# matwilso/generative_models

Measured on AMD Instinct MI355X. Metric: ddpm_train_images_per_sec, higher is better.
Workload: dtype fp16_fwd+bf16_bwd

## Files before the change

### generative_models_amd/csrc/conv_halo.hip

```cpp
#include "gmk_common.h"


namespace {

typedef __attribute__((ext_vector_type(4))) unsigned int u32x4;
typedef __attribute__((ext_vector_type(2))) unsigned int u32x2_t;

constexpr int kHaloSlots = 448;
constexpr int kHB = kHaloSlots * 128;
constexpr int kWOFF = 2 * kHB;
constexpr int kWST = 16384;

struct HaloParams {
    const void* src0; const void* src1;
    int c0, c1, ktot;
    int B, H, W, WE, R, TP, ntiles, rows_total;
    int nfull, nhalf;
    int shift;
    int pmask;
    const void* w; unsigned w_tap_stride_b; int n0;
    const float* bias; const float* emb; int emb_stride;
    const void* residual; void* out; int out_cstride; int M;
    unsigned nb0, nb1, nbw, nbo;
    const float* gn_scale; const float* gn_shift; int gn_stride;
// ... 1514 lines not shown
                if (tap < 8) pre(hbuf, tap + 1);
                if (tap == 8 && ph + 1 == nph) b_off = next_boff;
                if (kPrefetchW) load_wt(st, 0, 0);
                mfma_group(1, IntTag<0>{});
                if (tap < 8) interleave_pre();
                __builtin_amdgcn_sched_barrier(0);
            }
            hbuf ^= 1;
        };
        phase(IntTag<1>{}, 0);
        for (int ph = 1; ph < nph; ++ph) phase(IntTag<0>{}, ph);
        asm volatile("" ::: "memory");
        if (hand) {
            Rl = smem + (hbuf ^ 1) * HB;
            if (cwe == 1) {
#pragma unroll
                for (int i = 0; i < 4; ++i) {
                    const int ml = pxbase + i * 32 + r;
                    const int m = tile * p.TP + ml;
                    const unsigned off = (ml < p.TP && m < p.M) ? (unsigned)m * (unsigned)p.out_cstride * ES + (unsigned)(nblk + 112 + 8 * h) * ES : kBadOff;
                    r7[i] = __builtin_bit_cast(u32x4, __builtin_amdgcn_raw_buffer_load_b128(rsr, off, 0, 0));
                }
            }
            __builtin_amdgcn_s_barrier();
            __builtin_amdgcn_s_barrier();
        }
        epilogue();
    };

    set_geometry(job_half(0));
    b_off = WOFF + (cwe * 64 + r) * 128;
    resolve_centres(job_tile(0));
#pragma unroll
    for (int j = 0; j < 2; ++j)
#pragma unroll
        for (int i = 0; i < 4; ++i)
#pragma unroll
            for (int e = 0; e < 16; ++e) acc[j][i][e] = 0.f;
    __builtin_amdgcn_s_barrier();
    if (kPrefetchW) load_wt(0, 0, 0);
    for (int k = 0; k < njobs; ++k) {
        const int tile = job_tile(k), hc = job_half(k), ntile = job_tile(k + 1), nhc = job_half(k + 1);
        const int next_boff = WOFF + ((nhc >= 0 ? nhc : cw) * 64 + r) * 128;
        if (hc < 0) run_job(IntTag<4>{}, tile, next_boff);
        else run_job(IntTag<2>{}, tile, next_boff);
        if (nhc != hc) set_geometry(nhc);
        resolve_centres(ntile);
        asm volatile("" ::: "memory");
    }
}

}

static unsigned* g_stamps = nullptr;
static int64_t g_stamp_bytes = 0;
extern "C" int gmk_dev_set_stamp_buffer(void* buf, int64_t bytes) { g_stamps = (unsigned*)buf; g_stamp_bytes = bytes; return 0; }

int gmk_halo_geometry(int B, int H, int W, int c0, int c1, int w_rows, int cout, int out_cstride, int min_tiles, int upsample,
                      int fused_gn, HaloGeometry* g) {
    if (c0 % 64 || c1 % 64 || cout % 128) return 0;
    if (c1 != 0 && c1 != c0) return 0;
    if (W < 4 || W > 254 || H < 2) return 0;
    const int R = 256 / W;
    if (R < 1) return 0;
    const int crossings = H % R == 0 ? 0 : (R - 1 + H - 1) / H;
    const int ner = R + 2 + 2 * crossings;
    if (ner * (W + 2) > kHaloSlots) return 0;
    const int64_t rows_total = (int64_t)B * H;
    const int64_t M = rows_total * W;
    if (upsample && ((H | W) & 1)) return 0;
    const int64_t Msrc = upsample ? M / 4 : M;
    const int64_t nb0 = Msrc * c0 * 2, nb1 = Msrc * c1 * 2;
    const int64_t nbw = (int64_t)9 * w_rows * (c0 + c1) * 2, nbo = M * out_cstride * 2;
    const int64_t lim = 0xFFFF0000ll;
    if (nb0 >= lim || nb1 >= lim || nbw >= lim || nbo >= lim || M >= 0x00FFFFFF || c0 > 2048 || c1 > 2048) return 0;
    const int64_t ntiles = (rows_total + R - 1) / R;
    if (ntiles < min_tiles) return 0;
    if (fused_gn && (upsample || R > H)) return 0;
    if (g) {
        g->R = R; g->TP = R * W; g->slots = ner * (W + 1) + 1; g->rows_total = rows_total; g->M = M; g->ntiles = ntiles;
        g->nb0 = nb0; g->nb1 = nb1; g->nbw = nbw; g->nbo = nbo;
    }
    return 1;
}

int gmk_conv3x3_halo_try(const void* src0, const void* src1, int c0, int c1, int B, int H, int W, const void* w, int w_rows,
                         int n0, int cout, const float* bias, const float* emb, int emb_stride, const void* residual,
                         void* out, int out_cstride, int min_tiles, int upsample, float* stats, int64_t stats_bytes,
                         const float* gn_scale, const float* gn_shift, int gn_stride, int dtype, hipStream_t stream) {
    HaloGeometry g;
    if (!gmk_halo_geometry(B, H, W, c0, c1, w_rows, cout, out_cstride, min_tiles, upsample, gn_scale != nullptr, &g)) return 0;
    if (gn_scale && (!gn_shift || gn_stride < c0 + c1)) return 0;
    const int R = g.R, TP = g.TP;
    const int64_t rows_total = g.rows_total, M = g.M, ntiles = g.ntiles;
    const int64_t nb0 = g.nb0, nb1 = g.nb1, nbw = g.nbw, nbo = g.nbo;
    HaloParams p;
    p.src0 = src0; p.src1 = src1; p.c0 = c0; p.c1 = c1; p.ktot = c0 + c1;
    p.shift = upsample ? 1 : 0; p.pmask = upsample == 2 ? 1 : 0;
    p.B = B; p.H = H; p.W = W; p.WE = W + 1; p.R = R; p.TP = TP; p.ntiles = (int)ntiles; p.rows_total = (int)rows_total;
    p.w = w; p.w_tap_stride_b = (unsigned)w_rows * (unsigned)(c0 + c1) * 2u; p.n0 = n0;
    p.bias = bias; p.emb = emb; p.emb_stride = emb_stride; p.residual = residual; p.out = out; p.out_cstride = out_cstride;
    p.M = (int)M;
    p.nb0 = (unsigned)nb0; p.nb1 = (unsigned)nb1; p.nbw = (unsigned)nbw; p.nbo = (unsigned)nbo;
    p.gn_scale = gn_scale; p.gn_shift = gn_shift; p.gn_stride = gn_stride;
    p.stats = nullptr; p.stats_groups = out_cstride / 4; p.stamps = nullptr;
    p.variant = gmk_kernel_choice(3, "GMK_DEV_VARIANT") & 0xFF;
    if (stats && cout == out_cstride && stats_bytes >= ntiles * 8 * 2 * (int64_t)(out_cstride / 4) * 2 * 4 && H * W >= 32) p.stats = stats;
    p.inv_hp2 = 1.0f / (float)(H + 2); p.inv_h = 1.0f / (float)H; p.inv_we = 1.0f / (float)(W + 1); p.inv_w = 1.0f / (float)W;
    const int ncu = gmk_cu_limit();
// ... 93 lines not shown
```

### generative_models_amd/csrc/gmk_common.h

```cpp
#pragma once
#include <hip/hip_runtime.h>
#include <stdint.h>

#include "../../include/gmk.h"

typedef __bf16 bf16_t;
typedef __attribute__((ext_vector_type(8))) __bf16 bf16x8;
typedef __attribute__((ext_vector_type(4))) __bf16 bf16x4;
typedef _Float16 f16_t;
typedef __attribute__((ext_vector_type(8))) _Float16 f16x8;
typedef __attribute__((ext_vector_type(4))) _Float16 f16x4;
typedef __attribute__((ext_vector_type(2))) _Float16 f16x2;
typedef __attribute__((ext_vector_type(2))) __bf16 bf16x2;
typedef __attribute__((ext_vector_type(4))) short s16x4;
typedef __attribute__((ext_vector_type(4))) float f32x4;
typedef __attribute__((ext_vector_type(16))) float f32x16;

#define GMK_LDS __attribute__((address_space(3)))

void gmk_set_error(const char* fmt, ...);
int gmk_check_launch(const char* what);
int gmk_kernel_choice(int which, const char* env);
int gmk_conv1x1_pair_stream_try(const void* src, int64_t npix, const void* w_rows256, void* out_a, void* out_b, int dtype, hipStream_t stream);
int gmk_conv1x1_wgrad_stream_try(const void* dy, int dy_cstride, const void* src0, const void* src1, int64_t npix, float* slab, int64_t slab_bytes,
                                 bool x_f16, hipStream_t stream);
int gmk_conv_subpixel_takes(int B, int H, int W, int cin, int cout, int w_rows, int ntaps, int out_cstride, int dtype);
bool fp32_split(void);
int gmk_cu_limit(void);
void gmk_note_kernel(int id);

#define GMK_REQUIRE(cond, ...)                 \
    do {                                       \
        if (!(cond)) {                         \
            gmk_set_error(__VA_ARGS__);        \
            return GMK_ERR_ARG;                \
        }                                      \
    } while (0)

int gmk_conv3x3_halo_try(const void* src0, const void* src1, int c0, int c1, int B, int H, int W, const void* w, int w_rows,
                         int n0, int cout, const float* bias, const float* emb, int emb_stride, const void* residual,
                         void* out, int out_cstride, int min_tiles, int upsample, float* stats, int64_t stats_bytes,
                         const float* gn_scale, const float* gn_shift, int gn_stride, int dtype, hipStream_t stream);

struct HaloGeometry { int R, TP, slots; int64_t rows_total, M, ntiles, nb0, nb1, nbw, nbo; };
int gmk_halo_geometry(int B, int H, int W, int c0, int c1, int w_rows, int cout, int out_cstride, int min_tiles, int upsample,
                      int fused_gn, HaloGeometry* g);

int gmk_wgrad_slots_nsplit(int cout, int ktot);
int gmk_conv_wgrad_slots_try(const void* dy, int dy_cstride, const void* src0, const void* src1, int c0, int c1, int B, int H,
                             int W, int cout, float* slab, int64_t slab_bytes, int forced, int upsample, bool x_f16,
                             hipStream_t stream, int stride2 = 0);


static inline hipStream_t gmk_stream(void* s) { return reinterpret_cast<hipStream_t>(s); }
static inline int gmk_esize(int dtype) { return dtype == GMK_F32 ? 4 : 2; }
static inline bool gmk_is16(int dtype) { return dtype == GMK_BF16 || dtype == GMK_F16; }

template <typename T> struct Vec8;

__device__ __forceinline__ void load8(const float* p, float (&v)[8]) {
    const f32x4 a = *reinterpret_cast<const f32x4*>(p);
    const f32x4 b = *reinterpret_cast<const f32x4*>(p + 4);
    v[0] = a[0]; v[1] = a[1]; v[2] = a[2]; v[3] = a[3];
    v[4] = b[0]; v[5] = b[1]; v[6] = b[2]; v[7] = b[3];
}
__device__ __forceinline__ void load8(const bf16_t* p, float (&v)[8]) {
    const bf16x8 a = *reinterpret_cast<const bf16x8*>(p);
#pragma unroll
    for (int i = 0; i < 8; ++i) v[i] = (float)a[i];
}
__device__ __forceinline__ void load8(const f16_t* p, float (&v)[8]) {
    const f16x8 a = *reinterpret_cast<const f16x8*>(p);
#pragma unroll
    for (int i = 0; i < 8; ++i) v[i] = (float)a[i];
}
__device__ __forceinline__ void store8(float* p, const float (&v)[8]) {
    f32x4 a = {v[0], v[1], v[2], v[3]}, b = {v[4], v[5], v[6], v[7]};
    *reinterpret_cast<f32x4*>(p) = a;
    *reinterpret_cast<f32x4*>(p + 4) = b;
}
__device__ __forceinline__ void store8(bf16_t* p, const float (&v)[8]) {
    bf16x8 a;
// ... 121 lines not shown
```

### generative_models_amd/csrc/gmk_common.hip

```cpp
#include <stdarg.h>
#include <stdio.h>
#include <stdlib.h>

#include "gmk_common.h"

static thread_local char g_err[512] = "";

void gmk_set_error(const char* fmt, ...) {
    va_list ap;
    va_start(ap, fmt);
    vsnprintf(g_err, sizeof(g_err), fmt, ap);
    va_end(ap);
}

int gmk_check_launch(const char* what) {
    hipError_t e = hipGetLastError();
    if (e != hipSuccess) {
        gmk_set_error("%s: %s", what, hipGetErrorString(e));
        return (int)e;
    }
    return 0;
}

extern "C" int gmk_version(void) { return 1; }
extern "C" const char* gmk_last_error(void) { return g_err; }

static thread_local int g_last_kernel = 0;
void gmk_note_kernel(int id) { g_last_kernel = id; }
extern "C" int gmk_last_kernel(void) { return g_last_kernel; }

static int g_choice[4] = {-1, -1, -1, -1};
extern "C" int gmk_set_kernel_choice(int conv, int wgrad, int gn) {
    g_choice[0] = conv; g_choice[1] = wgrad; g_choice[2] = gn;
    return 0;
}
extern "C" int gmk_set_dev_variant(int v) { g_choice[3] = v; return 0; }
int gmk_kernel_choice(int which, const char* env) {
    if (g_choice[which] >= 0) return g_choice[which];
    const char* v = getenv(env);
    return v ? atoi(v) : 0;
}

static int g_cu_limit = -1;
extern "C" int gmk_set_cu_limit(int n) {
    if (n < 8 || n > 256) { gmk_set_error("gmk_set_cu_limit: %d not in [8, 256]", n); return GMK_ERR_ARG; }
    g_cu_limit = n;
    return 0;
}
int gmk_cu_limit(void) {
    if (g_cu_limit > 0) return g_cu_limit;
    const char* v = getenv("GMK_CU_LIMIT");
    const int n = v ? atoi(v) : 256;
    return n >= 8 && n <= 256 ? n : 256;
}
extern "C" int gmk_get_cu_limit(void) { return gmk_cu_limit(); }

static int g_fp32_exact = -1;
extern "C" int gmk_set_fp32_exact(int exact) { g_fp32_exact = exact ? 1 : 0; return 0; }
bool fp32_split(void) {
    if (g_fp32_exact < 0) {
        const char* v = getenv("GMK_FP32_SPLIT");
        g_fp32_exact = (v && atoi(v) != 0) ? 0 : 1;
    }
    return g_fp32_exact == 0;
}
extern "C" int gmk_fp32_split(void) { return fp32_split() ? 1 : 0; }
```

### generative_models_amd/csrc/gn_silu.hip

```cpp
#include <stdlib.h>

#include "gmk_common.h"

namespace {

constexpr int kThreads = 256;

__device__ __forceinline__ void drop8(float (&v)[8], size_t e0, float p, uint64_t seed, uint64_t off) {
    const float scale = 1.0f / (1.0f - p);
#pragma unroll
    for (int q = 0; q < 2; ++q) {
        uint32_t r[4];
        philox4x32(off + (uint64_t)(e0 >> 2) + q, seed, r);
#pragma unroll
        for (int k = 0; k < 4; ++k) v[4 * q + k] = u01(r[k]) >= p ? v[4 * q + k] * scale : 0.f;
    }
}

__device__ __forceinline__ void slab_of_block(int idx, int nslab, int B, int& b, int& slab) {
    if ((B & 7) == 0) {
        const int xcd = idx & 7, j = idx >> 3;
        slab = j % nslab;
        b = (j / nslab) * 8 + xcd;
    } else {
// ... 578 lines not shown
    } else
#pragma unroll
    for (int i = 0; i < ITER; ++i, eoff += estride, loff += PL * NVEC * 16) {
        if (ITER > 8) asm volatile("" : "+v"(eoff), "+v"(loff));
        const int p = pl + PL * i;
        if (!kExact && p >= HW) continue;
        const size_t off = eoff;
        const u32x4_t xr = i >= XLDS ? xk[i >= XLDS ? i - XLDS : 0] : *reinterpret_cast<const u32x4_t*>(xs_lds + loff);
        const u32x4_t dq2 = i < KEEP ? dr[i < KEEP ? i : 0] : *reinterpret_cast<const u32x4_t*>(dy + off);
        float o[8];
#pragma unroll
        for (int jj = 0; jj < 4; ++jj) {
            const f32x2_t xv = unpack2<TX>(xr[jj]), dv = unpack2<bf16_t>(dq2[jj]);
            const f32x2_t dg = silu_grad2(xv, dv, sv[jj], tv[jj], kNegLog2e);
            const f32x2_t ov = __builtin_elementwise_fma(dg, sv[jj], __builtin_elementwise_fma(xv, npv[jj], qv[jj]));
            o[2 * jj] = ov[0]; o[2 * jj + 1] = ov[1];
        }
        if (dadd1) {
            float t[8];
            load8(dadd1 + off, t);
#pragma unroll
            for (int k = 0; k < 8; ++k) o[k] += t[k];
        }
        if (dadd2) {
            float t[8];
            load8(dadd2 + off, t);
#pragma unroll
            for (int k = 0; k < 8; ++k) o[k] += t[k];
        }
#pragma unroll
        for (int k = 0; k < 8; ++k) xs[k] += o[k];
        store8(dx + off, o);
        if (i & 1) __builtin_amdgcn_sched_barrier(0);
    }
    if (dxsum) {
#pragma unroll
        for (int k = 0; k < 8; ++k) xs[k] = vec_lane_sum<NVEC>(xs[k]);
        __syncthreads();
        if (lane < NVEC) {
#pragma unroll
            for (int k = 0; k < 8; ++k) red[wave][lane][k] = xs[k];
        }
        __syncthreads();
        if (tid < CS) {
            const int vv = tid >> 3, k = tid & 7;
            float a = 0.f;
#pragma unroll
            for (int w = 0; w < NW; ++w) a += red[w][vv][k];
            dxsum[(size_t)b * dxsum_stride + c0 + tid] = a;
        }
    }
}

int gn_reg_iter(int HW, int nvec) {
    if (nvec == 8 && HW == 784 && gmk_kernel_choice(2, "GMK_GN_KERNEL") != 6) return 14;
    for (int it = 1; it <= 16; it <<= 1)
        if (((HW + it - 1) / it) * nvec <= 512) return it;
    return 0;
}


template <typename T>
__global__ __launch_bounds__(kThreads) void chansum_kernel(const T* __restrict__ x, float* __restrict__ out,
                                                          int out_stride, int HW, int C) {
    __shared__ float red[kThreads * 8];
    const int b = blockIdx.x, tid = threadIdx.x;
    const int nvec = C >> 3, planes = kThreads / nvec;
    const int vec = tid % nvec, pl = tid / nvec;
    const T* xb = x + (size_t)b * HW * C + vec * 8;
    float s[8];
#pragma unroll
    for (int i = 0; i < 8; ++i) s[i] = 0.f;
    for (int p = pl; p < HW; p += planes) {
        float v[8];
        load8(xb + (size_t)p * C, v);
#pragma unroll
        for (int i = 0; i < 8; ++i) s[i] += v[i];
    }
#pragma unroll
    for (int i = 0; i < 8; ++i) red[tid * 8 + i] = s[i];
    __syncthreads();
    if (tid < C) {
        const int vv = tid >> 3, i = tid & 7;
        float a = 0.f;
        for (int p = 0; p < planes; ++p) a += red[(p * nvec + vv) * 8 + i];
        out[(size_t)b * out_stride + tid] = a;
    }
}

__global__ __launch_bounds__(256) void colsum_kernel(const float* __restrict__ part, int64_t stride,
                                                    float* __restrict__ out, int R, int C, int accumulate) {
    __shared__ float red[8][33];
    const int cl = threadIdx.x & 31, rl = threadIdx.x >> 5;
    const int c = blockIdx.x * 32 + cl;
    float s = 0.f;
    if (c < C) {
        float s0 = 0.f, s1 = 0.f, s2 = 0.f, s3 = 0.f;
        int r = rl;
        for (; r + 24 < R; r += 32) {
            s0 += part[(int64_t)r * stride + c];
            s1 += part[(int64_t)(r + 8) * stride + c];
            s2 += part[(int64_t)(r + 16) * stride + c];
            s3 += part[(int64_t)(r + 24) * stride + c];
        }
        for (; r < R; r += 8) s0 += part[(int64_t)r * stride + c];
        s = (s0 + s1) + (s2 + s3);
// ... 32 lines not shown
        load8(p00 + (int64_t)2 * W * C + C, t);
#pragma unroll
        for (int i = 0; i < 8; ++i) a[i] += t[i];
        store8(y + ((b * H + oy) * W + ox) * (int64_t)C + vec * 8, a);
    }
}

template <typename TS, typename TD>
__global__ __launch_bounds__(256) void cast16_kernel(const TS* __restrict__ src, TD* __restrict__ dst, int64_t nvec) {
    fp16_saturating_stores<TD>();
    for (int64_t i = (int64_t)blockIdx.x * 256 + threadIdx.x; i < nvec; i += (int64_t)gridDim.x * 256) {
        float v[8];
        load8(src + i * 8, v);
#pragma unroll
        for (int k = 0; k < 8; ++k) v[k] = sat16<TD>(v[k]);
        store8(dst + i * 8, v);
    }
}

bool gn_shape_ok(int C, int G) {
    if (C <= 0 || C > 256 || (C & 7) || 256 % (C >> 3)) return false;
    if (G < 0) return -G >= 1 && -G <= 16;
    if (G <= 0 || G > 256 || C % G) return false;
    const int cpg = C / G;
    return cpg == 1 || cpg == 2 || cpg == 4 || cpg == 8 || cpg == 16;
}
static bool gn_narrow(int C, int G) { return G < 0 || C / G < 4; }

int gn_slab_channels(int mode, int C, int G, int HW, int elem_bytes, bool backward) {
    if (G < 0) return C;
    const int cpg = C / G;
    int CS = C;
    if (mode == 3) CS = 32;
    else if (mode == 4) CS = 64;
    else if (mode != 1) CS = backward && (int64_t)HW * C * elem_bytes > 65536 ? 32 : C;
    if (CS > C || C % CS || CS % cpg || (CS & 7) || kThreads % (CS >> 3)) CS = C;
    return CS;
}

}

extern "C" int gmk_gn_silu_fwd(const void* x, void* y, const float* gamma, const float* beta, float* mean, float* rstd,
                               int B, int HW, int C, int groups, float eps, const float* stats_part, int tile_pixels,
                               int ntiles, float drop_p, uint64_t drop_seed, uint64_t drop_offset, const float* xadd,
                               int xadd_stride, int dtype, void* stream) {
    GMK_REQUIRE(!xadd || xadd_stride >= C, "gmk_gn_silu_fwd: xadd_stride %d < C %d", xadd_stride, C);
    if (xadd) stats_part = nullptr;
    GMK_REQUIRE(drop_p >= 0.f && drop_p < 1.f, "gmk_gn_silu_fwd: dropout probability %g outside [0, 1)", (double)drop_p);
    GMK_REQUIRE(!stats_part || (tile_pixels >= 32 && ntiles > 0 && HW >= 32 && C % 4 == 0),
                "gmk_gn_silu_fwd: bad statistics geometry");
    GMK_REQUIRE(x && y && gamma && beta && mean && rstd, "gmk_gn_silu_fwd: null pointer");
    GMK_REQUIRE(B > 0 && HW > 0 && gn_shape_ok(C, groups), "gmk_gn_silu_fwd: unsupported shape B=%d HW=%d C=%d G=%d", B,
                HW, C, groups);
    const int gn_mode = gmk_kernel_choice(2, "GMK_GN_KERNEL");
    GMK_REQUIRE(dtype != GMK_F16 || !stats_part, "gmk_gn_silu_fwd: producer statistics go with bf16 tensors only");
    if (gn_narrow(C, groups)) {
        GMK_REQUIRE(!stats_part, "gmk_gn_silu_fwd: producer statistics come in 4-channel units; groups of %d channels", groups < 0 ? -groups : C / groups);
        gmk_note_kernel(22);
        if (dtype == GMK_BF16)
            gn_silu_fwd_kernel<bf16_t, true><<<B, kThreads, 0, gmk_stream(stream)>>>((const bf16_t*)x, (bf16_t*)y, gamma, beta, mean, rstd, HW, C, groups,
                                                                                   eps, nullptr, 0, 0, C, B, drop_p, drop_seed, drop_offset, xadd, xadd_stride);
        else if (dtype == GMK_F16)
            gn_silu_fwd_kernel<f16_t, true><<<B, kThreads, 0, gmk_stream(stream)>>>((const f16_t*)x, (f16_t*)y, gamma, beta, mean, rstd, HW, C, groups,
                                                                                  eps, nullptr, 0, 0, C, B, drop_p, drop_seed, drop_offset, xadd, xadd_stride);
        else if (dtype == GMK_F32)
            gn_silu_fwd_kernel<float, true><<<B, kThreads, 0, gmk_stream(stream)>>>((const float*)x, (float*)y, gamma, beta, mean, rstd, HW, C, groups,
                                                                                  eps, nullptr, 0, 0, C, B, drop_p, drop_seed, drop_offset, xadd, xadd_stride);
        else
            GMK_REQUIRE(false, "gmk_gn_silu_fwd: bad dtype %d", dtype);
        return gmk_check_launch("gmk_gn_silu_fwd");
    }
    const bool big = gmk_is16(dtype) && !stats_part && (gn_mode == 8 || gn_mode == 0) && HW > 1024 && HW <= 4096 && HW % 16 == 0 &&
                     C % 32 == 0 && 32 % (C / groups) == 0;
    if (big || (gmk_is16(dtype) && !stats_part && (gn_mode == 5 || gn_mode == 6 || (gn_mode == 0 && HW > 64)) && C % 64 == 0 &&
               32 % (C / groups) == 0 && gn_reg_iter(HW, 8) > 0)) {
        const int nvec = (big || gn_mode == 5) ? 4 : 8;
        const int it = big ? 16 : gn_reg_iter(HW, nvec), planes = (HW + it - 1) / it, threads = (planes * nvec + 63) / 64 * 64;
        const int nblk = B * (C / (nvec * 8));
        gmk_note_kernel(21);
#define GMK_GN_FWD_REG(IT, NV)                                                                                                           \
    do {                                                                                                                                 \
        if (dtype == GMK_F16)                                                                                                            \
            gn_silu_fwd_reg_kernel<f16_t, IT, NV><<<nblk, threads, 0, gmk_stream(stream)>>>((const f16_t*)x, (f16_t*)y, gamma, beta, mean, rstd, \
                                                                                            HW, C, groups, eps, B, planes, drop_p, drop_seed,  \
                                                                                            drop_offset, xadd, xadd_stride);                   \
        else                                                                                                                             \
            gn_silu_fwd_reg_kernel<bf16_t, IT, NV><<<nblk, threads, 0, gmk_stream(stream)>>>((const bf16_t*)x, (bf16_t*)y, gamma, beta, mean,  \
                                                                                             rstd, HW, C, groups, eps, B, planes, drop_p,      \
                                                                                             drop_seed, drop_offset, xadd, xadd_stride);       \
    } while (0)
        if (nvec == 4) {
            if (it == 1) GMK_GN_FWD_REG(1, 4);
            else if (it == 2) GMK_GN_FWD_REG(2, 4);
            else if (it == 4) GMK_GN_FWD_REG(4, 4);
            else if (it == 8) GMK_GN_FWD_REG(8, 4);
            else GMK_GN_FWD_REG(16, 4);
        } else {
            if (it == 1) GMK_GN_FWD_REG(1, 8);
            else if (it == 2) GMK_GN_FWD_REG(2, 8);
            else if (it == 4) GMK_GN_FWD_REG(4, 8);
            else if (it == 8) GMK_GN_FWD_REG(8, 8);
            else if (it == 14) GMK_GN_FWD_REG(14, 8);
            else GMK_GN_FWD_REG(16, 8);
        }
#undef GMK_GN_FWD_REG
    } else if (dtype == GMK_BF16) {
        gmk_note_kernel(22);
// ... 42 lines not shown
        else                                                                                                                              \
            gn_silu_fwd_reg_kernel<bf16_t, IT, 8><<<nblk, threads, 0, gmk_stream(stream)>>>((const bf16_t*)x, (bf16_t*)nullptr, gamma, beta,     \
                                                                                            mean, rstd, HW, C, groups, eps, B, planes, 0.f, 0, 0, \
                                                                                            xadd, xadd_stride, tab_scale, tab_shift, tab_stride); \
    } while (0)
        if (it == 1) GMK_GN_STATS_REG(1);
        else if (it == 2) GMK_GN_STATS_REG(2);
        else if (it == 4) GMK_GN_STATS_REG(4);
        else if (it == 8) GMK_GN_STATS_REG(8);
        else if (it == 14) GMK_GN_STATS_REG(14);
        else GMK_GN_STATS_REG(16);
#undef GMK_GN_STATS_REG
    } else if (HW > 1024 && HW <= 4096 && HW % 16 == 0 && C % 32 == 0 && 32 % (C / groups) == 0) {
        const int planes = HW / 16, nblk = B * (C / 32);
        gmk_note_kernel(21);
        if (dtype == GMK_F16)
            gn_silu_fwd_reg_kernel<f16_t, 16, 4><<<nblk, planes * 4, 0, gmk_stream(stream)>>>((const f16_t*)x, (f16_t*)nullptr, gamma, beta, mean, rstd,
                                                                                             HW, C, groups, eps, B, planes, 0.f, 0, 0, xadd, xadd_stride,
                                                                                             tab_scale, tab_shift, tab_stride);
        else
            gn_silu_fwd_reg_kernel<bf16_t, 16, 4><<<nblk, planes * 4, 0, gmk_stream(stream)>>>((const bf16_t*)x, (bf16_t*)nullptr, gamma, beta, mean, rstd,
                                                                                              HW, C, groups, eps, B, planes, 0.f, 0, 0, xadd, xadd_stride,
                                                                                              tab_scale, tab_shift, tab_stride);
    } else {
        const int CS = gn_slab_channels(0, C, groups, HW, 2, false);
        gmk_note_kernel(22);
        if (dtype == GMK_F16)
            gn_silu_fwd_kernel<f16_t><<<B * (C / CS), kThreads, 0, gmk_stream(stream)>>>(
                (const f16_t*)x, (f16_t*)nullptr, gamma, beta, mean, rstd, HW, C, groups, eps, nullptr, 0, 0, CS, B, 0.f, 0, 0, xadd,
                xadd_stride, tab_scale, tab_shift, tab_stride);
        else
            gn_silu_fwd_kernel<bf16_t><<<B * (C / CS), kThreads, 0, gmk_stream(stream)>>>(
                (const bf16_t*)x, (bf16_t*)nullptr, gamma, beta, mean, rstd, HW, C, groups, eps, nullptr, 0, 0, CS, B, 0.f, 0, 0, xadd,
                xadd_stride, tab_scale, tab_shift, tab_stride);
    }
    return gmk_check_launch("gmk_gn_stats");
}

extern "C" int gmk_gn_silu_bwd(const void* dy, const void* x, const float* gamma, const float* beta, const float* mean,
                               const float* rstd, const void* dadd1, const void* dadd2, void* dx, float* dgamma_part,
                               float* dbeta_part, float* dxsum, int dxsum_stride, int B, int HW, int C, int groups,
                               float drop_p, uint64_t drop_seed, uint64_t drop_offset, const float* xadd, int xadd_stride,
                               int dtype, int x_dtype, void* stream) {
    GMK_REQUIRE(!xadd || xadd_stride >= C, "gmk_gn_silu_bwd: xadd_stride %d < C %d", xadd_stride, C);
    GMK_REQUIRE(x_dtype == dtype || (dtype == GMK_BF16 && x_dtype == GMK_F16),
                "gmk_gn_silu_bwd: x of type %d with gradients of type %d (same type, or fp16 activations with bf16 gradients)", x_dtype, dtype);
    const bool xf16 = x_dtype == GMK_F16;
    GMK_REQUIRE(drop_p >= 0.f && drop_p < 1.f, "gmk_gn_silu_bwd: dropout probability %g outside [0, 1)", (double)drop_p);
    GMK_REQUIRE(dy && x && gamma && beta && mean && rstd && dx && dgamma_part && dbeta_part,
                "gmk_gn_silu_bwd: null pointer");
    GMK_REQUIRE(B > 0 && HW > 0 && gn_shape_ok(C, groups), "gmk_gn_silu_bwd: unsupported shape B=%d HW=%d C=%d G=%d", B,
                HW, C, groups);
    GMK_REQUIRE(!dxsum || dxsum_stride >= C, "gmk_gn_silu_bwd: dxsum_stride %d < C %d", dxsum_stride, C);
    const int gn_mode = gn_narrow(C, groups) ? 1 : gmk_kernel_choice(2, "GMK_GN_KERNEL");
    if (dtype == GMK_BF16 && (gn_mode == 0 || gn_mode == 7) && C % 32 == 0 && 32 % (C / groups) == 0 && HW > (gn_mode == 7 ? 511 : 64) &&
               HW <= 1024 && drop_p == 0.f) {
        const size_t lds = (size_t)HW * 64;
        gmk_note_kernel(23);
#define GMK_GN_BWD_HYB(IT, TH)                                                                                                          \
    do {                                                                                                                                \
        if (xf16)                                                                                                                       \
            gn_silu_bwd_hybrid_kernel<f16_t, IT, TH><<<B * (C / 32), TH, lds, gmk_stream(stream)>>>(                                     \
                (const bf16_t*)dy, (const f16_t*)x, gamma, beta, mean, rstd, (const bf16_t*)dadd1, (const bf16_t*)dadd2, (bf16_t*)dx,     \
                dgamma_part, dbeta_part, dxsum, dxsum_stride, HW, C, groups, B, drop_p, drop_seed, drop_offset, xadd, xadd_stride);   \
        else                                                                                                                            \
            gn_silu_bwd_hybrid_kernel<bf16_t, IT, TH><<<B * (C / 32), TH, lds, gmk_stream(stream)>>>(                                    \
                (const bf16_t*)dy, (const bf16_t*)x, gamma, beta, mean, rstd, (const bf16_t*)dadd1, (const bf16_t*)dadd2, (bf16_t*)dx,    \
                dgamma_part, dbeta_part, dxsum, dxsum_stride, HW, C, groups, B, drop_p, drop_seed, drop_offset, xadd, xadd_stride);   \
    } while (0)
        if (HW == 1024) {
            if (xf16)
                gn_silu_bwd_hybrid_kernel<f16_t, 8, 512, 4, 8, 0, true><<<B * (C / 32), 512, lds, gmk_stream(stream)>>>(
                    (const bf16_t*)dy, (const f16_t*)x, gamma, beta, mean, rstd, (const bf16_t*)dadd1, (const bf16_t*)dadd2, (bf16_t*)dx,
                    dgamma_part, dbeta_part, dxsum, dxsum_stride, HW, C, groups, B, drop_p, drop_seed, drop_offset, xadd, xadd_stride);
            else
                gn_silu_bwd_hybrid_kernel<bf16_t, 8, 512, 4, 8, 0, true><<<B * (C / 32), 512, lds, gmk_stream(stream)>>>(
                    (const bf16_t*)dy, (const bf16_t*)x, gamma, beta, mean, rstd, (const bf16_t*)dadd1, (const bf16_t*)dadd2, (bf16_t*)dx,
                    dgamma_part, dbeta_part, dxsum, dxsum_stride, HW, C, groups, B, drop_p, drop_seed, drop_offset, xadd, xadd_stride);
        } else
        if (HW <= 256) GMK_GN_BWD_HYB(4, 256);
        else if (HW <= 832) GMK_GN_BWD_HYB(13, 256);
        else GMK_GN_BWD_HYB(8, 512);
#undef GMK_GN_BWD_HYB
    } else if (dtype == GMK_BF16 && (gn_mode == 0 || gn_mode == 9) && C % 32 == 0 && 32 % (C / groups) == 0 && HW == 4096 && drop_p == 0.f) {
        gmk_note_kernel(23);
        constexpr int kParkBytes = 19 * 128 * 64;
        static const hipError_t attr = hipFuncSetAttribute((const void*)gn_silu_bwd_hybrid_kernel<bf16_t, 32, 512, 4, 28, 13>,
                                                           hipFuncAttributeMaxDynamicSharedMemorySize, kParkBytes);
        static const hipError_t attr16 = hipFuncSetAttribute((const void*)gn_silu_bwd_hybrid_kernel<f16_t, 32, 512, 4, 28, 13>,
                                                             hipFuncAttributeMaxDynamicSharedMemorySize, kParkBytes);
        (void)attr; (void)attr16;
        if (xf16)
            gn_silu_bwd_hybrid_kernel<f16_t, 32, 512, 4, 28, 13><<<B * (C / 32), 512, kParkBytes, gmk_stream(stream)>>>(
                (const bf16_t*)dy, (const f16_t*)x, gamma, beta, mean, rstd, (const bf16_t*)dadd1, (const bf16_t*)dadd2, (bf16_t*)dx,
                dgamma_part, dbeta_part, dxsum, dxsum_stride, HW, C, groups, B, drop_p, drop_seed, drop_offset, xadd, xadd_stride);
        else
            gn_silu_bwd_hybrid_kernel<bf16_t, 32, 512, 4, 28, 13><<<B * (C / 32), 512, kParkBytes, gmk_stream(stream)>>>(
                (const bf16_t*)dy, (const bf16_t*)x, gamma, beta, mean, rstd, (const bf16_t*)dadd1, (const bf16_t*)dadd2, (bf16_t*)dx,
                dgamma_part, dbeta_part, dxsum, dxsum_stride, HW, C, groups, B, drop_p, drop_seed, drop_offset, xadd, xadd_stride);
    } else if (dtype == GMK_BF16 && (gn_mode == 0 || gn_mode == 7) && C % 16 == 0 && 16 % (C / groups) == 0 && HW > 1024 &&
               HW <= 4096 && drop_p == 0.f) {
        gmk_note_kernel(23);
        static const hipError_t attr = hipFuncSetAttribute((const void*)gn_silu_bwd_hybrid_kernel<bf16_t, 8, 1024, 2>,
                                                           hipFuncAttributeMaxDynamicSharedMemorySize, 4096 * 32);
        static const hipError_t attr16 = hipFuncSetAttribute((const void*)gn_silu_bwd_hybrid_kernel<f16_t, 8, 1024, 2>,
                                                             hipFuncAttributeMaxDynamicSharedMemorySize, 4096 * 32);
        (void)attr; (void)attr16;
        if (xf16)
            gn_silu_bwd_hybrid_kernel<f16_t, 8, 1024, 2><<<B * (C / 16), 1024, (size_t)HW * 32, gmk_stream(stream)>>>(
                (const bf16_t*)dy, (const f16_t*)x, gamma, beta, mean, rstd, (const bf16_t*)dadd1, (const bf16_t*)dadd2, (bf16_t*)dx,
                dgamma_part, dbeta_part, dxsum, dxsum_stride, HW, C, groups, B, drop_p, drop_seed, drop_offset, xadd, xadd_stride);
        else
            gn_silu_bwd_hybrid_kernel<bf16_t, 8, 1024, 2><<<B * (C / 16), 1024, (size_t)HW * 32, gmk_stream(stream)>>>(
                (const bf16_t*)dy, (const bf16_t*)x, gamma, beta, mean, rstd, (const bf16_t*)dadd1, (const bf16_t*)dadd2, (bf16_t*)dx,
                dgamma_part, dbeta_part, dxsum, dxsum_stride, HW, C, groups, B, drop_p, drop_seed, drop_offset, xadd, xadd_stride);
    } else if (dtype == GMK_BF16 && xf16) {
        gmk_note_kernel(24);
        const int CS = gn_slab_channels(gn_mode, C, groups, HW, 2, true);
        gn_silu_bwd_kernel<bf16_t, f16_t><<<B * (C / CS), kThreads, 0, gmk_stream(stream)>>>(
            (const bf16_t*)dy, (const f16_t*)x, gamma, beta, mean, rstd, (const bf16_t*)dadd1, (const bf16_t*)dadd2,
            (bf16_t*)dx, dgamma_part, dbeta_part, dxsum, dxsum_stride, HW, C, groups, CS, B, drop_p, drop_seed, drop_offset, xadd,
            xadd_stride);
    } else if (dtype == GMK_BF16) {
// ... 67 lines not shown
```

### generative_models_amd/ops.py

```python
import math

import os

import torch

from ._lib import check, lib

F32, BF16, F16 = 0, 1, 2
_DT = {torch.float32: F32, torch.bfloat16: BF16, torch.float16: F16}
_HALF = (torch.bfloat16, torch.float16)
NORMAL, STRIDE2, UPSAMPLE2, TRANSPOSED2 = 0, 1, 2, 3

PROFILE = None


KERNEL_NAMES = {1: "conv_igemm_kernel", 2: "conv_igemm_dma_kernel", 3: "conv3x3_halo_kernel", 4: "conv3x3_halo_ws_kernel", 11: "conv_wgrad_kernel",
                12: "conv_wgrad_slots_kernel", 13: "conv_wgrad_slots_ws_kernel", 16: "conv_wgrad_subpixel_ws_kernel", 14: "conv1x1_pair_stream_kernel", 15: "conv1x1_wgrad_stream_kernel",
                5: "conv3x3_halo_ws_kernel[zero-stuffed transposed conv]",
                7: "conv3x3_halo_ws_kernel[+1x1 skip]",
                6: "conv_igemm_dma_kernel[stride-2 dgrad phases]",
                17: "conv_wgrad_slots_ws_kernel[stride-2 planes]",
                8: "conv_subpixel_ws_kernel[upsample]", 9: "conv_subpixel_ws_kernel[transposed]", 10: "conv_subpixel_ws_kernel[upsample dgrad]",
                21: "gn_silu_fwd_reg_kernel", 22: "gn_silu_fwd_kernel", 23: "gn_silu_bwd_hybrid_kernel", 24: "gn_silu_bwd_kernel"}


def instantiation_key(name, dtype):
    if dtype not in _HALF:
        return None
    t = "f16" if dtype == torch.float16 else "bf16"
    if name == "conv3x3_halo_ws_kernel":
        return f"{name}<{t}>"
    if name == "conv3x3_halo_ws_kernel[+1x1 skip]":
        return f"conv3x3_halo_ws_kernel<{t},+skip>"
    if name == "conv_wgrad_slots_ws_kernel[stride-2 planes]":
        return "conv_wgrad_slots_ws_kernel<stride-2 planes>"
    if name.startswith("conv_subpixel_ws_kernel["):
        return f"conv_subpixel_ws_kernel<{t},{name[len('conv_subpixel_ws_kernel['):-1]}>"
    return None


def _nbytes(*tensors):
    if PROFILE is None:
        return 0.0
    return float(sum(t.numel() * t.element_size() for t in tensors if t is not None))


class _Timed:

    def __init__(self, name, flops, nbytes=0.0, fixed=False, multiplied=None, dtype=None):
        self.on = PROFILE is not None
        if self.on:
            self.name, self.flops, self.nbytes, self.fixed = name, flops, nbytes, fixed
            self.multiplied = flops if multiplied is None else multiplied
            self.dtype = dtype
            self.s = torch.cuda.Event(enable_timing=True)
            self.e = torch.cuda.Event(enable_timing=True)

    def __enter__(self):
        if self.on:
            self.s.record()

    def __exit__(self, *exc):
        if self.on:
            self.e.record()
            name = self.name if self.fixed else KERNEL_NAMES.get(lib.gmk_last_kernel(), self.name)
            PROFILE.append((name, self.s, self.e, self.flops, self.nbytes, self.multiplied, instantiation_key(name, self.dtype)))


_IN_FLIGHT = {}


def throttle(max_in_flight=2):
    q = _IN_FLIGHT.setdefault(torch.cuda.current_device(), [])
    ev = torch.cuda.Event()
    ev.record()
    q.append(ev)
# ... 743 lines not shown
```

Baseline: 46420.

## Add burst-load GroupNorm+SiLU backward kernel for 1024-pixel slabs

Adds a specialized GN+SiLU backward kernel for HW=1024 that issues all x/dy buffer loads up front (LEAD=8), keeps dy in registers and x in LDS, and prefetches gradient addends in double-buffered pairs during the second pass. It replaces the generic hybrid kernel on the default path and removes per-slab reloads of dy from memory. The larger register footprint is pinned to 4 waves per EU, which may limit occupancy. Optional memtime stamping instrumentation is also added, with the stamp buffer globals moved to common code.

```diff
diff --git a/generative_models_amd/csrc/conv_halo.hip b/generative_models_amd/csrc/conv_halo.hip
--- a/generative_models_amd/csrc/conv_halo.hip
+++ b/generative_models_amd/csrc/conv_halo.hip
@@ -1590,9 +1590,6 @@
 
 }
 
-static unsigned* g_stamps = nullptr;
-static int64_t g_stamp_bytes = 0;
-extern "C" int gmk_dev_set_stamp_buffer(void* buf, int64_t bytes) { g_stamps = (unsigned*)buf; g_stamp_bytes = bytes; return 0; }
 
 int gmk_halo_geometry(int B, int H, int W, int c0, int c1, int w_rows, int cout, int out_cstride, int min_tiles, int upsample,
                       int fused_gn, HaloGeometry* g) {
diff --git a/generative_models_amd/csrc/gmk_common.h b/generative_models_amd/csrc/gmk_common.h
--- a/generative_models_amd/csrc/gmk_common.h
+++ b/generative_models_amd/csrc/gmk_common.h
@@ -28,6 +28,8 @@
 bool fp32_split(void);
 int gmk_cu_limit(void);
 void gmk_note_kernel(int id);
+extern unsigned* g_stamps;
+extern int64_t g_stamp_bytes;
 
 #define GMK_REQUIRE(cond, ...)                 \
     do {                                       \
diff --git a/generative_models_amd/csrc/gmk_common.hip b/generative_models_amd/csrc/gmk_common.hip
--- a/generative_models_amd/csrc/gmk_common.hip
+++ b/generative_models_amd/csrc/gmk_common.hip
@@ -28,6 +28,10 @@
 static thread_local int g_last_kernel = 0;
 void gmk_note_kernel(int id) { g_last_kernel = id; }
 extern "C" int gmk_last_kernel(void) { return g_last_kernel; }
+
+unsigned* g_stamps = nullptr;
+int64_t g_stamp_bytes = 0;
+extern "C" int gmk_dev_set_stamp_buffer(void* buf, int64_t bytes) { g_stamps = (unsigned*)buf; g_stamp_bytes = bytes; return 0; }
 
 static int g_choice[4] = {-1, -1, -1, -1};
 extern "C" int gmk_set_kernel_choice(int conv, int wgrad, int gn) {
diff --git a/generative_models_amd/csrc/gn_silu.hip b/generative_models_amd/csrc/gn_silu.hip
--- a/generative_models_amd/csrc/gn_silu.hip
+++ b/generative_models_amd/csrc/gn_silu.hip
@@ -654,6 +654,251 @@
     }
 }
 
+constexpr int waitcnt_vm(int n) { return (n & 15) | (7 << 4) | (15 << 8) | ((n >> 4) << 14); }
+__device__ __forceinline__ void wait_vm(int n) {
+    switch (n) {
+#define GMK_WAIT_VM(k) case k: __builtin_amdgcn_s_waitcnt(waitcnt_vm(k)); break;
+        GMK_WAIT_VM(0) GMK_WAIT_VM(1) GMK_WAIT_VM(2) GMK_WAIT_VM(3) GMK_WAIT_VM(4) GMK_WAIT_VM(5) GMK_WAIT_VM(6) GMK_WAIT_VM(7)
+        GMK_WAIT_VM(8) GMK_WAIT_VM(9) GMK_WAIT_VM(10) GMK_WAIT_VM(11) GMK_WAIT_VM(12) GMK_WAIT_VM(13) GMK_WAIT_VM(14)
+#undef GMK_WAIT_VM
+        default: __builtin_amdgcn_s_waitcnt(waitcnt_vm(0));
+    }
+}
+
+template <typename TX, int NADD, int LEAD, bool kStamp>
+__global__ __launch_bounds__(512) __attribute__((amdgpu_waves_per_eu(4, 4))) void gn_silu_bwd_burst_kernel(
+    const bf16_t* __restrict__ dy, const TX* __restrict__ x, const float* __restrict__ gamma, const float* __restrict__ beta,
+    const float* __restrict__ mean, const float* __restrict__ rstd, const bf16_t* __restrict__ dadd1, const bf16_t* __restrict__ dadd2,
+    bf16_t* __restrict__ dx, float* __restrict__ dgp, float* __restrict__ dbp, float* __restrict__ dxsum, int dxsum_stride, int C, int G, int B,
+    const float* __restrict__ xadd, int xadd_stride, unsigned* __restrict__ stamps) {
+    constexpr int HW = 1024, NVEC = 4, CS = 32, ITER = 8, NW = 8, PL = 128;
+    static_assert(LEAD >= 1 && LEAD <= ITER, "LEAD: 1 .. 8 pixels");
+    static_assert(NADD >= 0 && NADD <= 2, "NADD: 0 .. 2 gradient addends (dadd1, then dadd2)");
+    extern __shared__ __attribute__((aligned(16))) char xs_lds[];
+    __shared__ float red[NW][NVEC][16];
+    __shared__ float chg[CS], chb[CS];
+    __shared__ float sA[8], sB[8], gam[CS];
+    const int tid = threadIdx.x, lane = tid & 63, wave = tid >> 6;
+    const int vec = tid & (NVEC - 1), pl = tid / NVEC;
+    int b, slab;
+    slab_of_block(blockIdx.x, C / CS, B, b, slab);
+    uint64_t st_t = 0, st_p = 0;
+    unsigned st[8] = {0u, 0u, 0u, 0u, 0u, 0u, 0u, 0u};
+    if constexpr (kStamp) { st_t = __builtin_amdgcn_s_memtime(); st_p = st_t; __builtin_amdgcn_sched_barrier(0); }
+    const int cpg = C / G, c0 = slab * CS, g0 = c0 / cpg, gps = CS / cpg;
+    const int glo = (vec * 8) / cpg, ghi = (vec * 8 + 4) / cpg;
+    const int nbytes = HW * C * 2;
+    const size_t sbase = (size_t)b * HW * C;
+    const __amdgpu_buffer_rsrc_t rsx = __builtin_amdgcn_make_buffer_rsrc(const_cast<TX*>(x + sbase), 0, nbytes, 0x00020000);
+    const __amdgpu_buffer_rsrc_t rsd = __builtin_amdgcn_make_buffer_rsrc(const_cast<bf16_t*>(dy + sbase), 0, nbytes, 0x00020000);
+    const __amdgpu_buffer_rsrc_t rs1 = __builtin_amdgcn_make_buffer_rsrc(const_cast<bf16_t*>(dadd1 ? dadd1 + sbase : dy), 0, nbytes, 0x00020000);
+    const __amdgpu_buffer_rsrc_t rs2 = __builtin_amdgcn_make_buffer_rsrc(const_cast<bf16_t*>(dadd2 ? dadd2 + sbase : dy), 0, nbytes, 0x00020000);
+    bf16_t* const dxw = dx + sbase + (size_t)pl * C + c0 + vec * 8;
+    const int voff = (pl * C + c0 + vec * 8) * 2, sstep = PL * C * 2;
+    const float rs0 = rstd[b * G + g0 + glo], rs1v = rstd[b * G + g0 + ghi];
+    const float mu0 = mean[b * G + g0 + glo], mu1 = mean[b * G + g0 + ghi];
+    float pa[8], pg[8], pb[8];
+#pragma unroll
+    for (int k = 0; k < 8; ++k) {
+        const int c = c0 + vec * 8 + k;
+        pa[k] = xadd ? xadd[(size_t)b * xadd_stride + c] : 0.f;
+        pg[k] = gamma[c]; pb[k] = beta[c];
+    }
+    __builtin_amdgcn_sched_barrier(0);
+    u32x4_t xr[ITER], dr[ITER];
+#pragma unroll
+    for (int i = 0; i < LEAD; ++i) {
+        xr[i] = __builtin_amdgcn_raw_buffer_load_b128(rsx, voff, i * sstep, 0);
+        dr[i] = __builtin_amdgcn_raw_buffer_load_b128(rsd, voff, i * sstep, 0);
+    }
+    __builtin_amdgcn_sched_barrier(0);
+    f32x2_t sv[4], tv[4], muv[4];
+#pragma unroll
+    for (int jj = 0; jj < 4; ++jj) {
+#pragma unroll
+        for (int e = 0; e < 2; ++e) {
+            const int k = 2 * jj + e;
+            const float m = (k < 4 ? mu0 : mu1) - pa[k], sc = (k < 4 ? rs0 : rs1v) * pg[k];
+            muv[jj][e] = m; sv[jj][e] = sc; tv[jj][e] = pb[k] - m * sc;
+        }
+    }
+    constexpr float kNegLog2e = -1.4426950408889634f;
+    f32x2_t ax[4], ab[4];
+#pragma unroll
+    for (int jj = 0; jj < 4; ++jj) { ax[jj] = f32x2_t{0.f, 0.f}; ab[jj] = f32x2_t{0.f, 0.f}; }
+    const uint32_t loff = ((uint32_t)pl * NVEC + vec) * 16;
+#pragma unroll
+    for (int i = 0; i < ITER; ++i) {
+        if (i + LEAD < ITER) {
+            xr[i + LEAD] = __builtin_amdgcn_raw_buffer_load_b128(rsx, voff, (i + LEAD) * sstep, 0);
+            dr[i + LEAD] = __builtin_amdgcn_raw_buffer_load_b128(rsd, voff, (i + LEAD) * sstep, 0);
+        }
+        if constexpr (kStamp) {
+            __builtin_amdgcn_sched_barrier(0);
+            const uint64_t t0 = __builtin_amdgcn_s_memtime();
+            wait_vm(2 * ((i + LEAD + 1 < ITER ? i + LEAD + 1 : ITER) - i - 1));
+            const uint64_t t1 = __builtin_amdgcn_s_memtime();
+            st[0] += (unsigned)(t1 - t0);
+            __builtin_amdgcn_sched_barrier(0);
+        }
+        const u32x4_t xq = xr[i], dv4 = dr[i];
+        *reinterpret_cast<u32x4_t*>(xs_lds + loff + i * (PL * NVEC * 16)) = xq;
+#pragma unroll
+        for (int jj = 0; jj < 4; ++jj) {
+            const f32x2_t xv = unpack2<TX>(xq[jj]), dv = unpack2<bf16_t>(dv4[jj]);
+            const f32x2_t dg = silu_grad2(xv, dv, sv[jj], tv[jj], kNegLog2e);
+            ax[jj] = __builtin_elementwise_fma(dg, xv, ax[jj]);
+            ab[jj] += dg;
+        }
+#pragma unroll
+        for (int jj = 0; jj < 4; ++jj) asm volatile("" : "+v"(ax[jj]), "+v"(ab[jj]));
+        __builtin_amdgcn_sched_barrier(0);
+    }
+    u32x4_t a1[2][2], a2[2][2];
+#pragma unroll
+    for (int u = 0; u < 2; ++u) {
+        if (NADD > 0) a1[0][u] = __builtin_amdgcn_raw_buffer_load_b128(rs1, voff, u * sstep, 0);
+        if (NADD > 1) a2[0][u] = __builtin_amdgcn_raw_buffer_load_b128(rs2, voff, u * sstep, 0);
+    }
+    if constexpr (kStamp) {
+        __builtin_amdgcn_sched_barrier(0);
+        const uint64_t t = __builtin_amdgcn_s_memtime();
+        st[1] = (unsigned)(t - st_p) - st[0]; st_p = t;
+        __builtin_amdgcn_sched_barrier(0);
+    }
+#pragma unroll
+    for (int i = 0; i < ITER; ++i) asm volatile("" : "+v"(dr[i]));
+    float ag[8], abk[8];
+#pragma unroll
+    for (int jj = 0; jj < 4; ++jj) {
+#pragma unroll
+        for (int e = 0; e < 2; ++e) {
+            const int k = 2 * jj + e;
+            abk[k] = ab[jj][e];
+            ag[k] = (ax[jj][e] - muv[jj][e] * ab[jj][e]) * (k < 4 ? rs0 : rs1v);
+        }
+    }
+#pragma unroll
+    for (int k = 0; k < 8; ++k) { ag[k] = vec_lane_sum<NVEC>(ag[k]); abk[k] = vec_lane_sum<NVEC>(abk[k]); }
+    if (lane < NVEC) {
+#pragma unroll
+        for (int k = 0; k < 8; ++k) { red[wave][lane][k] = ag[k]; red[wave][lane][8 + k] = abk[k]; }
+        if (wave == 0) {
+#pragma unroll
+            for (int k = 0; k < 8; ++k) gam[lane * 8 + k] = pg[k];
+        }
+    }
+    __syncthreads();
+    if (tid < CS) {
+        const int vv = tid >> 3, k = tid & 7;
+        float a = 0.f, bb = 0.f;
+#pragma unroll
+        for (int w = 0; w < NW; ++w) { a += red[w][vv][k]; bb += red[w][vv][8 + k]; }
+        chg[tid] = a; chb[tid] = bb;
+        dgp[(size_t)b * C + c0 + tid] = a;
+        dbp[(size_t)b * C + c0 + tid] = bb;
+    }
+    __syncthreads();
+    if (tid < gps) {
+        float A = 0.f, Bq = 0.f;
+        for (int j = 0; j < cpg; ++j) {
+            const int cl = tid * cpg + j;
+            A = fmaf(gam[cl], chb[cl], A);
+            Bq = fmaf(gam[cl], chg[cl], Bq);
+        }
+        const float inv_n = 1.f / ((float)cpg * (float)HW);
+        sA[tid] = A * inv_n; sB[tid] = Bq * inv_n;
+    }
+    __syncthreads();
+    f32x2_t npv[4], qv[4];
+#pragma unroll
+    for (int jj = 0; jj < 4; ++jj) {
+        const float rsk = jj < 2 ? rs0 : rs1v, cA = jj < 2 ? sA[glo] : sA[ghi], cB = jj < 2 ? sB[glo] : sB[ghi];
+        const float r2b = rsk * rsk * cB;
+        npv[jj] = f32x2_t{-r2b, -r2b};
+        qv[jj] = muv[jj] * r2b - rsk * cA;
+    }
+    if constexpr (kStamp) {
+        __builtin_amdgcn_sched_barrier(0);
+        const uint64_t t = __builtin_amdgcn_s_memtime();
+        st[2] = (unsigned)(t - st_p); st_p = t;
+        __builtin_amdgcn_sched_barrier(0);
+    }
+    float xs[8];
+#pragma unroll
+    for (int k = 0; k < 8; ++k) xs[k] = 0.f;
+    constexpr int N2 = ITER / 2;
+#pragma unroll
+    for (int c = 0; c < N2; ++c) {
+        if (c + 1 < N2) {
+#pragma unroll
+            for (int u = 0; u < 2; ++u) {
+                const int i = 2 * (c + 1) + u;
+                if (NADD > 0) a1[(c + 1) & 1][u] = __builtin_amdgcn_raw_buffer_load_b128(rs1, voff, i * sstep, 0);
+                if (NADD > 1) a2[(c + 1) & 1][u] = __builtin_amdgcn_raw_buffer_load_b128(rs2, voff, i * sstep, 0);
+            }
+            __builtin_amdgcn_sched_barrier(0);
+        }
+#pragma unroll
+        for (int u = 0; u < 2; ++u) {
+            const int i = 2 * c + u;
+            const u32x4_t xq = *reinterpret_cast<const u32x4_t*>(xs_lds + loff + i * (PL * NVEC * 16));
+            const u32x4_t dv4 = dr[i];
+            u32x4_t ow;
+#pragma unroll
+            for (int jj = 0; jj < 4; ++jj) {
+                const f32x2_t xv = unpack2<TX>(xq[jj]), dv = unpack2<bf16_t>(dv4[jj]);
+                const f32x2_t dg = silu_grad2(xv, dv, sv[jj], tv[jj], kNegLog2e);
+                f32x2_t ov = __builtin_elementwise_fma(dg, sv[jj], __builtin_elementwise_fma(xv, npv[jj], qv[jj]));
+                if (NADD > 0) ov += unpack2<bf16_t>(a1[c & 1][u][jj]);
+                if (NADD > 1) ov += unpack2<bf16_t>(a2[c & 1][u][jj]);
+                xs[2 * jj] += ov[0]; xs[2 * jj + 1] += ov[1];
+                ow[jj] = pack_pair<bf16_t>(ov[0], ov[1]);
+            }
+            *reinterpret_cast<u32x4_t*>(dxw + (size_t)i * PL * C) = ow;
+        }
+#pragma unroll
+        for (int k = 0; k < 8; ++k) asm volatile("" : "+v"(xs[k]));
+        __builtin_amdgcn_sched_barrier(0);
+    }
+    if constexpr (kStamp) {
+        const uint64_t t = __builtin_amdgcn_s_memtime();
+        st[3] = (unsigned)(t - st_p); st_p = t;
+        __builtin_amdgcn_sched_barrier(0);
+        __builtin_amdgcn_s_waitcnt(waitcnt_vm(0));
+        const uint64_t t1 = __builtin_amdgcn_s_memtime();
+        st[4] = (unsigned)(t1 - st_p); st_p = t1;
+        __builtin_amdgcn_sched_barrier(0);
+    }
+    if (dxsum) {
+#pragma unroll
+        for (int k = 0; k < 8; ++k) xs[k] = vec_lane_sum<NVEC>(xs[k]);
+        __syncthreads();
+        if (lane < NVEC) {
+#pragma unroll
+            for (int k = 0; k < 8; ++k) red[wave][lane][k] = xs[k];
+        }
+        __syncthreads();
+        if (tid < CS) {
+            const int vv = tid >> 3, k = tid & 7;
+            float a = 0.f;
+#pragma unroll
+            for (int w = 0; w < NW; ++w) a += red[w][vv][k];
+            dxsum[(size_t)b * dxsum_stride + c0 + tid] = a;
+        }
+    }
+    if constexpr (kStamp) {
+        __builtin_amdgcn_sched_barrier(0);
+        const uint64_t t = __builtin_amdgcn_s_memtime();
+        st[5] = (unsigned)(t - st_p);
+        st[6] = (unsigned)(t - st_t);
+        if (tid == 0) {
+#pragma unroll
+            for (int k = 0; k < 8; ++k) stamps[(size_t)blockIdx.x * 8 + k] = st[k];
+        }
+    }
+}
+
 int gn_reg_iter(int HW, int nvec) {
     if (nvec == 8 && HW == 784 && gmk_kernel_choice(2, "GMK_GN_KERNEL") != 6) return 14;
     for (int it = 1; it <= 16; it <<= 1)
@@ -792,7 +1037,8 @@
     GMK_REQUIRE(x && y && gamma && beta && mean && rstd, "gmk_gn_silu_fwd: null pointer");
     GMK_REQUIRE(B > 0 && HW > 0 && gn_shape_ok(C, groups), "gmk_gn_silu_fwd: unsupported shape B=%d HW=%d C=%d G=%d", B,
                 HW, C, groups);
-    const int gn_mode = gmk_kernel_choice(2, "GMK_GN_KERNEL");
+    int gn_mode = gmk_kernel_choice(2, "GMK_GN_KERNEL");
+    if (gn_mode == 10) gn_mode = 0;
     GMK_REQUIRE(dtype != GMK_F16 || !stats_part, "gmk_gn_silu_fwd: producer statistics go with bf16 tensors only");
     if (gn_narrow(C, groups)) {
         GMK_REQUIRE(!stats_part, "gmk_gn_silu_fwd: producer statistics come in 4-channel units; groups of %d channels", groups < 0 ? -groups : C / groups);
@@ -941,7 +1187,9 @@
     GMK_REQUIRE(B > 0 && HW > 0 && gn_shape_ok(C, groups), "gmk_gn_silu_bwd: unsupported shape B=%d HW=%d C=%d G=%d", B,
                 HW, C, groups);
     GMK_REQUIRE(!dxsum || dxsum_stride >= C, "gmk_gn_silu_bwd: dxsum_stride %d < C %d", dxsum_stride, C);
-    const int gn_mode = gn_narrow(C, groups) ? 1 : gmk_kernel_choice(2, "GMK_GN_KERNEL");
+    int gn_mode = gn_narrow(C, groups) ? 1 : gmk_kernel_choice(2, "GMK_GN_KERNEL");
+    const bool hybrid32 = gn_mode == 10;
+    if (hybrid32) gn_mode = 0;
     if (dtype == GMK_BF16 && (gn_mode == 0 || gn_mode == 7) && C % 32 == 0 && 32 % (C / groups) == 0 && HW > (gn_mode == 7 ? 511 : 64) &&
                HW <= 1024 && drop_p == 0.f) {
         const size_t lds = (size_t)HW * 64;
@@ -957,7 +1205,36 @@
                 (const bf16_t*)dy, (const bf16_t*)x, gamma, beta, mean, rstd, (const bf16_t*)dadd1, (const bf16_t*)dadd2, (bf16_t*)dx,    \
                 dgamma_part, dbeta_part, dxsum, dxsum_stride, HW, C, groups, B, drop_p, drop_seed, drop_offset, xadd, xadd_stride);   \
     } while (0)
-        if (HW == 1024) {
+        if (HW == 1024 && gn_mode == 0 && !hybrid32) {
+            gmk_note_kernel(25);
+            const bool stamp = g_stamps && g_stamp_bytes >= (int64_t)B * (C / 32) * 32;
+            const bool lead2 = stamp && gmk_kernel_choice(3, "GMK_DEV_VARIANT") == 2;
+            const void* a1 = dadd1 ? dadd1 : dadd2;
+            const void* a2 = dadd1 ? dadd2 : nullptr;
+            const int nadd = (a1 != nullptr) + (a2 != nullptr);
+#define GMK_GN_BWD_BURST(TX, NADD, LEAD, ST)                                                                                            \
+    gn_silu_bwd_burst_kernel<TX, NADD, LEAD, ST><<<B * (C / 32), 512, lds, gmk_stream(stream)>>>(                                      \
+        (const bf16_t*)dy, (const TX*)x, gamma, beta, mean, rstd, (const bf16_t*)a1, (const bf16_t*)a2, (bf16_t*)dx, dgamma_part,      \
+        dbeta_part, dxsum, dxsum_stride, C, groups, B, xadd, xadd_stride, g_stamps)
+#define GMK_GN_BWD_BURST_N(TX, LEAD, ST)                                                                                                \
+    do {                                                                                                                                \
+        if (nadd == 0) GMK_GN_BWD_BURST(TX, 0, LEAD, ST);                                                                              \
+        else if (nadd == 1) GMK_GN_BWD_BURST(TX, 1, LEAD, ST);                                                                         \
+        else GMK_GN_BWD_BURST(TX, 2, LEAD, ST);                                                                                        \
+    } while (0)
+            if (!stamp) {
+                if (xf16) GMK_GN_BWD_BURST_N(f16_t, 8, false);
+                else GMK_GN_BWD_BURST_N(bf16_t, 8, false);
+            } else if (lead2) {
+                if (xf16) GMK_GN_BWD_BURST_N(f16_t, 2, true);
+                else GMK_GN_BWD_BURST_N(bf16_t, 2, true);
+            } else {
+                if (xf16) GMK_GN_BWD_BURST_N(f16_t, 8, true);
+                else GMK_GN_BWD_BURST_N(bf16_t, 8, true);
+            }
+#undef GMK_GN_BWD_BURST_N
+#undef GMK_GN_BWD_BURST
+        } else if (HW == 1024) {
             if (xf16)
                 gn_silu_bwd_hybrid_kernel<f16_t, 8, 512, 4, 8, 0, true><<<B * (C / 32), 512, lds, gmk_stream(stream)>>>(
                     (const bf16_t*)dy, (const f16_t*)x, gamma, beta, mean, rstd, (const bf16_t*)dadd1, (const bf16_t*)dadd2, (bf16_t*)dx,
diff --git a/generative_models_amd/ops.py b/generative_models_amd/ops.py
--- a/generative_models_amd/ops.py
+++ b/generative_models_amd/ops.py
@@ -21,7 +21,8 @@
                 6: "conv_igemm_dma_kernel[stride-2 dgrad phases]",
                 17: "conv_wgrad_slots_ws_kernel[stride-2 planes]",
                 8: "conv_subpixel_ws_kernel[upsample]", 9: "conv_subpixel_ws_kernel[transposed]", 10: "conv_subpixel_ws_kernel[upsample dgrad]",
-                21: "gn_silu_fwd_reg_kernel", 22: "gn_silu_fwd_kernel", 23: "gn_silu_bwd_hybrid_kernel", 24: "gn_silu_bwd_kernel"}
+                21: "gn_silu_fwd_reg_kernel", 22: "gn_silu_fwd_kernel", 23: "gn_silu_bwd_hybrid_kernel", 24: "gn_silu_bwd_kernel",
+                25: "gn_silu_bwd_burst_kernel"}
 
 
 def instantiation_key(name, dtype):
```

New measurement: 46870, median of 6. Within noise of the previous version (+1.0%).
